# hellobertrand/zxc

Hardware: AMD Instinct MI355X
Metric: seekable decode GB/s (level 3, 64 KiB independent blocks, HBM-resident in/out) (higher is better)
Workload: dtype u8

## Files before the change

### zxc_amd/csrc/zxc_decode_kernel.hip

```cpp
#include "zxc_experiments.h"
#include <hip/hip_runtime.h>
#include <stdint.h>

#include "zxc_kernels.h"
#include "zxc_wave.h"

typedef unsigned __int128 u128;

#include "zxc_lds.h"

#define RING_BYTES 4096u
#define RING_MASK (RING_BYTES - 1u)
#define RING_WORDS (RING_BYTES / 4u)
#define REDIRECT_PASSES 2
#define SPARSE_MAX 8
#define TILE_MAX 3584u
#define LIT_MED 128u
#define MATCH_MED 128u
#define BYTEWISE_MAX 32u

#define E_DST_TOO_SMALL (-2)
#define E_SRC_TOO_SMALL (-3)
#define E_BAD_HEADER (-6)
#define E_BAD_CHECKSUM (-7)
// ... 1053 lines not shown
        return r;
    const uint64_t consumed = (uint64_t)lit_comp + tok_comp + (uint64_t)n_seq * (enc_off ? 1u : 2u);
    if (consumed > avail || avail - lit_comp < 32u) return r;
    if (enc_tok == 2u && (n_seq == 0u || n_seq > block_size / 5u + 16u || n_seq > PDIR_N_MAX || tok_comp < 128u || pdir_class(tok_comp - 128u) > 2u))
        return r;
    r.cls = ZXC_DEV_CLS_PRE;
    if (enc_lit == 2u) {
        r.lit16 = (16u + n_lit + 64u + 15u) >> 4;
        r.lit_cls = pdir_class(lit_comp - 128u);
        r.lit_at = 8u + 12u + desc;
        r.lit_psize = lit_comp;
        r.n_lit = n_lit;
    }
    if (enc_tok == 2u) {
        r.tok16 = (n_seq + 64u + 15u) >> 4;
        r.tok_cls = pdir_class(tok_comp - 128u);
        r.tok_at = 8u + 12u + desc + lit_comp;
        r.tok_psize = tok_comp;
        r.n_seq = n_seq;
    }
    return r;
}

template <bool PRE>
__device__ __forceinline__ void lean_one_block(const uint8_t* __restrict__ comp, const zxc_dev_job_t* __restrict__ jobs,
                                               uint8_t* __restrict__ out, int32_t* __restrict__ status, uint32_t block_size,
                                               uint32_t cap_override, uint32_t trailer_bytes, uint32_t b,
                                               const zxc_dev_pre_t* __restrict__ pre, const uint8_t* __restrict__ pscratch, LeanLds& L,
                                               int lane, const uint8_t* __restrict__ rle_slot, int rle_rc) {
    const uint32_t cap = cap_override ? cap_override : block_size + 2112u;
    const bool ck_here = !(trailer_bytes & ZXC_DEV_TRAILER_ELSEWHERE);
    trailer_bytes &= ~ZXC_DEV_TRAILER_ELSEWHERE;
#ifdef EXP_TIMES
    const uint64_t t_start = wall_clock64();
#endif
    const uint64_t comp_off = jobs[b].comp_off;
    const uint32_t src_sz = uni(jobs[b].comp_size);
    const uint32_t out_len = uni(jobs[b].out_len);
    const uint8_t* src = comp + comp_off;
    uint8_t* dst = out + jobs[b].out_off;
    int rc;
    if (src_sz < 8u) {
        rc = E_SRC_TOO_SMALL;
    } else {
        const uint32_t type = uni(ld8(src));
        const uint32_t comp_sz = uni(ld32(src + 3));
        if ((uint64_t)8u + comp_sz + trailer_bytes > src_sz) {
            rc = E_SRC_TOO_SMALL;
        } else if (trailer_bytes && ck_here && wave_checksum32(src + 8, comp_sz, lane) != uni(ld32(src + 8 + comp_sz))) {
            rc = E_BAD_CHECKSUM;
        } else if (PRE) {
            rc = type == 1u ? decode_lz_block_lean(src + 8, comp_sz, false, dst, out_len, cap, L, lane, pre + b, pscratch, false) : ZXC_DEV_E_INTERNAL;
        } else if (type == 1u || type == 2u) {
            rc = rle_slot ? rle_rc : 0;
            if (rc == 0) rc = decode_lz_block_lean(src + 8, comp_sz, type == 2u, dst, out_len, cap, L, lane, nullptr, pscratch, false,
                                                   rle_slot ? rle_slot + 16 : nullptr, rle_slot != nullptr);
        } else if (type == 0u) {
            if (comp_sz > cap) rc = E_DST_TOO_SMALL;
            else {
                const uint32_t n = comp_sz < out_len ? comp_sz : out_len;
                const uint8_t* s8 = src + 8;
                uint32_t i = 16u * lane;
                for (; i + 3072u + 16u <= n; i += 4096u) {
                    const v4u a0 = ld128(s8 + i), a1 = ld128(s8 + i + 1024u), a2 = ld128(s8 + i + 2048u),
                              a3 = ld128(s8 + i + 3072u);
                    *(v4u*)(dst + i) = a0;
                    *(v4u*)(dst + i + 1024u) = a1;
                    *(v4u*)(dst + i + 2048u) = a2;
                    *(v4u*)(dst + i + 3072u) = a3;
                }
                for (; i + 16u <= n; i += 1024u) *(v4u*)(dst + i) = ld128(s8 + i);
                const uint32_t tail = n & ~15u;
                if (tail + (uint32_t)lane < n) dst[tail + lane] = s8[tail + lane];
                rc = (int)comp_sz;
            }
        } else if (type == 255u) {
            rc = E_CORRUPT;
        } else {
            rc = E_BAD_BLOCK_TYPE;
        }
    }
#ifdef EXP_TIMES
    __builtin_amdgcn_s_waitcnt(0);
    {
        const uint64_t t_end = wall_clock64();
        rc = (int)((((uint32_t)(t_start >> 5) & 0xFFFFu) << 16) | (uint32_t)(((t_end - t_start) >> 5) & 0xFFFFu));
    }
#endif
    if (lane == 0) status[b] = rc == ZXC_DEV_DEFER ? ZXC_DEV_E_INTERNAL : rc;
}

extern "C" __global__ void __launch_bounds__(64, LEAN_WAVES_PER_SIMD)
zxc_decode_blocks_lean_kernel(const uint8_t* __restrict__ comp, const zxc_dev_job_t* __restrict__ jobs, uint32_t n_jobs,
                              uint8_t* __restrict__ out, int32_t* __restrict__ status, uint32_t block_size,
                              const uint32_t* __restrict__ order, uint32_t cap_override, uint32_t trailer_bytes,
                              const zxc_dev_pre_t* __restrict__ pre, const uint8_t* __restrict__ rscratch) {
    __shared__ LeanLds L;
    if (blockIdx.x >= n_jobs) return;
    const uint32_t b = order ? uni(order[blockIdx.x]) : blockIdx.x;
    const uint32_t cls = uni(pre[b].cls);
    if (cls != ZXC_DEV_CLS_LEAN && cls != ZXC_DEV_CLS_LEAN_RLE) return;
    const uint8_t* rle_slot = cls == ZXC_DEV_CLS_LEAN_RLE ? rscratch + 16ull * uni(pre[b].lit_off) : nullptr;
    const int rle_rc = cls == ZXC_DEV_CLS_LEAN_RLE ? (int)(int16_t)uni((uint32_t)(uint16_t)pre[b].rc_lit) : 0;
    lean_one_block<false>(comp, jobs, out, status, block_size, cap_override, trailer_bytes, b, nullptr, nullptr, L, threadIdx.x, rle_slot, rle_rc);
}

extern "C" __global__ void __launch_bounds__(64)
zxc_rle_expand_kernel(const uint8_t* __restrict__ comp, const zxc_dev_job_t* __restrict__ jobs, zxc_dev_pre_t* __restrict__ pre,
                      uint8_t* __restrict__ rscratch, const uint32_t* __restrict__ hdr, const uint32_t* __restrict__ entries_last) {
    const int lane = threadIdx.x;
    const uint32_t n = uni(hdr[0]);
    for (uint32_t i = blockIdx.x; i < n; i += gridDim.x) {
        const uint32_t b = uni(*(entries_last - i));
        const uint8_t* src = comp + jobs[b].comp_off;
        const uint32_t n_lit = uni(ld32(src + 12));
        int rc = 0;
        if (n_lit != 0u) rc = rle_expand(src + 8 + 16, uni(ld32(src + 20)), rscratch + 16ull * uni(pre[b].lit_off) + 16u, n_lit, lane);
        if (lane == 0) pre[b].rc_lit = (int16_t)rc;
    }
}

extern "C" __global__ void __launch_bounds__(64, LEAN_WAVES_PER_SIMD)
zxc_decode_blocks_lean_pre_kernel(const uint8_t* __restrict__ comp, const zxc_dev_job_t* __restrict__ jobs, uint8_t* __restrict__ out,
                                  int32_t* __restrict__ status, uint32_t block_size, uint32_t cap_override, uint32_t trailer_bytes,
                                  const zxc_dev_pre_t* __restrict__ pre, const uint8_t* __restrict__ pscratch,
                                  const uint32_t* __restrict__ hdr, const uint32_t* __restrict__ entries) {
    __shared__ LeanLds L;
    if (blockIdx.x >= uni(hdr[0])) return;
    lean_one_block<true>(comp, jobs, out, status, block_size, cap_override, trailer_bytes, uni(entries[blockIdx.x]), pre, pscratch, L, threadIdx.x, nullptr, 0);
}

extern "C" __global__ void __launch_bounds__(64)
zxc_block_checksum_kernel(const uint8_t* __restrict__ comp, const zxc_dev_job_t* __restrict__ jobs, uint32_t n_jobs,
                          const uint32_t* __restrict__ order, uint8_t* __restrict__ ck_bad) {
    const int lane = threadIdx.x;
    const uint32_t slot = blockIdx.x * 9u + (uint32_t)lane / 7u;
    const bool in = lane < 63 && slot < n_jobs;
    const uint32_t b = in ? (order ? order[slot] : slot) : 0u;
    const uint8_t* src = comp + jobs[b].comp_off;
    const uint32_t src_sz = in ? jobs[b].comp_size : 0u;
    uint32_t comp_sz = 0;
    bool on = false;
    if (src_sz >= 8u) {
        comp_sz = ld32(src + 3);
        on = (uint64_t)8u + comp_sz + 4u <= src_sz;
    }
    const uint32_t h = group_checksum32(src + 8, on ? comp_sz : 0u, lane, on);
    if (on && lane % 7 == 0) ck_bad[b] = h != ld32(src + 8 + comp_sz) ? 1u : 0u;
    else if (in && !on && lane % 7 == 0) ck_bad[b] = 0u;
}
extern "C" __global__ void __launch_bounds__(256)
zxc_checksum_merge_kernel(const uint8_t* __restrict__ ck_bad, int32_t* __restrict__ status, uint32_t n_jobs) {
    const uint32_t i = blockIdx.x * 256u + threadIdx.x;
    if (i < n_jobs && ck_bad[i]) status[i] = E_BAD_CHECKSUM;
}

__device__ __forceinline__ uint32_t order_bucket(const uint8_t* __restrict__ comp, const zxc_dev_job_t& j, uint32_t block_size) {
    uint32_t cost = 0;
    if (j.comp_size >= 8u + 12u) {
        const uint8_t* h = comp + j.comp_off;
        const uint32_t type = ld8(h);
        if (type == 1u || type == 2u) {
            const uint32_t n_seq = ld32(h + 8), n_lit = ld32(h + 12), enc_lit = ld8(h + 16), enc_tok = ld8(h + 17);
            cost = n_seq + (enc_tok == 2u ? n_seq : 0u) + (enc_lit == 1u ? n_lit >> 4 : 0u) + (enc_lit >= 2u ? n_lit >> 2 : 0u);
        }
    }
    const uint64_t q = (uint64_t)cost * 320u / block_size;
    return 63u - (q > 63u ? 63u : (uint32_t)q);
}

extern "C" __global__ void __launch_bounds__(256)
zxc_order_hist_kernel(const uint8_t* __restrict__ comp, const zxc_dev_job_t* __restrict__ jobs, uint32_t n_jobs,
                      uint32_t block_size, uint32_t* __restrict__ hist) {
    __shared__ uint32_t cnt[64];
    if (threadIdx.x < 64u) cnt[threadIdx.x] = 0;
    __syncthreads();
    const uint32_t i = blockIdx.x * 256u + threadIdx.x;
    if (i < n_jobs) atomicAdd(cnt + order_bucket(comp, jobs[i], block_size), 1u);
    __syncthreads();
    if (threadIdx.x < 64u && cnt[threadIdx.x]) atomicAdd(hist + threadIdx.x, cnt[threadIdx.x]);
}

extern "C" __global__ void __launch_bounds__(256)
zxc_order_scatter_kernel(const uint8_t* __restrict__ comp, const zxc_dev_job_t* __restrict__ jobs, uint32_t n_jobs,
                         uint32_t block_size, uint32_t* __restrict__ hist, uint32_t* __restrict__ order,
                         uint32_t* __restrict__ list, uint32_t trailer_bytes, zxc_dev_pre_t* __restrict__ pre,
                         uint32_t* __restrict__ ctl, uint32_t* __restrict__ pre_entries, zxc_dev_sec_t* __restrict__ secs,
                         uint32_t pscratch_cap16, uint32_t cap, uint32_t rscratch_cap16) {
    __shared__ uint32_t cnt[64], base[64];
    __shared__ uint32_t wg_cnt[8], wg_base[8];
    __shared__ uint32_t wg_fit, wg_rle_fit;
    if (threadIdx.x < 64u) cnt[threadIdx.x] = 0;
    if (threadIdx.x < 8u) wg_cnt[threadIdx.x] = 0;
    __syncthreads();
    const uint32_t i = blockIdx.x * 256u + threadIdx.x;
    uint32_t bk = 0, rank = 0;
    if (i < n_jobs) {
        bk = order_bucket(comp, jobs[i], block_size);
        rank = atomicAdd(cnt + bk, 1u);
    }
    __syncthreads();
    if (threadIdx.x < 64u) {
        uint32_t s = 0;
        for (uint32_t k = 0; k < threadIdx.x; k++) s += hist[k];
        base[threadIdx.x] = cnt[threadIdx.x] ? s + atomicAdd(hist + 64u + threadIdx.x, cnt[threadIdx.x]) : 0u;
    }
    __syncthreads();
    if (i < n_jobs) order[base[bk] + rank] = i;
    if (!list) return;
    BlockClass c = {ZXC_DEV_CLS_LEAN, 0, 0, 3, 3, 0, 0, 0, 0, 0, 0};
    uint32_t my_off = 0, my_pre = 0, my_full = 0, my_lit = 0, my_tok = 0;
    if (i < n_jobs) {
        c = classify_block(comp + jobs[i].comp_off, jobs[i].comp_size, trailer_bytes, block_size, cap);
        if (c.cls == ZXC_DEV_CLS_PRE) {
            my_off = atomicAdd(wg_cnt + 0, c.lit16 + c.tok16);
            my_pre = atomicAdd(wg_cnt + 1, 1u);
            if (c.lit_cls < 3u) my_lit = atomicAdd(wg_cnt + 3u + c.lit_cls, 1u);
            if (c.tok_cls < 3u) my_tok = atomicAdd(wg_cnt + 3u + c.tok_cls, 1u);
        } else if (c.cls == ZXC_DEV_CLS_FULL) {
            my_full = atomicAdd(wg_cnt + 2, 1u);
        } else if (c.cls == ZXC_DEV_CLS_LEAN_RLE) {
            my_off = atomicAdd(wg_cnt + 6, c.lit16);
            my_pre = atomicAdd(wg_cnt + 7, 1u);
        }
    }
    __syncthreads();
    if (threadIdx.x == 0) {
        bool rfit = rscratch_cap16 != 0u;
        wg_base[6] = 0;
        if (wg_cnt[7]) {
            atomicAdd(ctl + ZXC_DEV_CTL_RLE_WANTED, wg_cnt[6] + 1u);
            if (wg_cnt[6]) {
// ... 11 lines not shown
        }
        wg_rle_fit = rfit ? 1u : 0u;
        bool fit = true;
        wg_base[0] = 0;
        if (wg_cnt[0]) {
            uint32_t old = __hip_atomic_load(ctl + ZXC_DEV_CTL_CURSOR, __ATOMIC_RELAXED, __HIP_MEMORY_SCOPE_AGENT);
            for (;;) {
                if (old > pscratch_cap16) { fit = false; break; }
                const uint32_t seen = atomicCAS(ctl + ZXC_DEV_CTL_CURSOR, old, old + wg_cnt[0]);
                if (seen == old) { fit = (uint64_t)old + wg_cnt[0] <= pscratch_cap16; break; }
                old = seen;
            }
            wg_base[0] = old;
        }
        wg_fit = fit ? 1u : 0u;
        if (wg_cnt[1]) atomicAdd(ctl + ZXC_DEV_CTL_WANTED, wg_cnt[1]);
        if (fit) {
            wg_base[1] = wg_cnt[1] ? atomicAdd(ctl + ZXC_DEV_CTL_PRE, wg_cnt[1]) : 0u;
            wg_base[2] = wg_cnt[2] ? atomicAdd(list, wg_cnt[2]) : 0u;
            for (uint32_t k = 0; k < 3u; k++) wg_base[3u + k] = wg_cnt[3u + k] ? atomicAdd(ctl + ZXC_DEV_CTL_SEC + 2u * k, wg_cnt[3u + k]) : 0u;
        } else {
            wg_base[2] = atomicAdd(list, wg_cnt[2] + wg_cnt[1]);
        }
    }
    __syncthreads();
    if (i >= n_jobs) return;
    uint32_t cls = c.cls;
    if (cls == ZXC_DEV_CLS_PRE && !wg_fit) {
        cls = ZXC_DEV_CLS_FULL;
        my_full = wg_cnt[2] + my_pre;
    }
    if (cls == ZXC_DEV_CLS_LEAN_RLE) {
        if (wg_rle_fit) {
            pre_entries[n_jobs - 1u - (wg_base[7] + my_pre)] = i;
            pre[i].lit_off = wg_base[6] + my_off;
            pre[i].tok_off = 0;
            pre[i].rc_lit = 0;
            pre[i].rc_tok = 0;
            pre[i].cls = cls;
            return;
        }
        cls = ZXC_DEV_CLS_FULL;
        my_full = wg_cnt[2] - wg_cnt[7] + my_pre;
    }
    const uint32_t off = wg_base[0] + my_off;
    pre[i].lit_off = off;
    pre[i].tok_off = off + c.lit16;
    pre[i].rc_lit = 0;
    pre[i].rc_tok = 0;
    pre[i].cls = cls;
    if (cls == ZXC_DEV_CLS_FULL) {
        list[2u + wg_base[2] + my_full] = base[bk] + rank;
    } else if (cls == ZXC_DEV_CLS_PRE) {
        pre_entries[wg_base[1] + my_pre] = i;
        if (c.lit_cls < 3u) {
            zxc_dev_sec_t& s = secs[(size_t)c.lit_cls * 2u * n_jobs + wg_base[3u + c.lit_cls] + my_lit];
            s.src_off = jobs[i].comp_off + c.lit_at;
            s.psize = c.lit_psize;
            s.n = c.n_lit;
            s.out_off4 = 4u * off + 4u;
            s.rc_slot = 8u * i + 4u;
        }
        if (c.tok_cls < 3u) {
            zxc_dev_sec_t& s = secs[(size_t)c.tok_cls * 2u * n_jobs + wg_base[3u + c.tok_cls] + my_tok];
            s.src_off = jobs[i].comp_off + c.tok_at;
            s.psize = c.tok_psize;
            s.n = c.n_seq;
            s.out_off4 = 4u * (off + c.lit16);
            s.rc_slot = 8u * i + 5u;
        }
    }
}
```

### zxc_amd/csrc/zxc_dev.h

```cpp
#ifndef ZXC_DEV_H
#define ZXC_DEV_H
#include "../../include/zxc_mi355x.h"

#define ZXC_DEV_E_UNSUPPORTED (-101)
#define ZXC_DEV_DEFER (-103)
#define ZXC_DEV_E_INTERNAL (-102)

#define ZXC_DEV_CLS_LEAN 0u
#define ZXC_DEV_CLS_FULL 1u
#define ZXC_DEV_CLS_PRE 2u
#define ZXC_DEV_CLS_LEAN_RLE 3u
typedef struct {
    uint32_t lit_off;
    uint32_t tok_off;
    int16_t rc_lit, rc_tok;
    uint32_t cls;
} zxc_dev_pre_t;
typedef struct {
    uint64_t src_off;
    uint32_t psize, n;
    uint32_t out_off4;
    uint32_t rc_slot;
    uint32_t pad[2];
} zxc_dev_sec_t;
#define ZXC_DEV_TRAILER_ELSEWHERE 0x80000000u
#define ZXC_DEV_CTL_WORDS 32u
#define ZXC_DEV_CTL_PRE 0u
#define ZXC_DEV_CTL_CURSOR 2u
#define ZXC_DEV_CTL_WANTED 3u
#define ZXC_DEV_CTL_SEC 4u
#define ZXC_DEV_CTL_RLE_CURSOR 10u
#define ZXC_DEV_CTL_RLE_WANTED 11u
#define ZXC_DEV_CTL_RLE_LIST 12u

#define ZXC_DEV_SLOT_REGION(bs) ((bs) + 64u)
#define ZXC_DEV_SLOT_STRIDE(bs) ((2u * ZXC_DEV_SLOT_REGION(bs) + (bs) / 5u + 16u + 64u + 255u) & ~255u)

typedef struct { size_t list, order, ctl, pre_ent, secs, pre, ck_bad, words; } zxc_dev_ord_layout_t;
static inline zxc_dev_ord_layout_t zxc_dev_ord_layout(uint32_t n_jobs) {
    const size_t n = n_jobs, ctl = 130u + 2u * n, pre_ent = ctl + ZXC_DEV_CTL_WORDS, secs = (pre_ent + n + 7u) & ~(size_t)7u;
    const zxc_dev_ord_layout_t l = {128u, 130u + n, ctl, pre_ent, secs, secs + 48u * n, secs + 52u * n, secs + 52u * n + (n + 3u) / 4u};
    return l;
}

enum { ZXC_DEV_PLAN_FULL, ZXC_DEV_PLAN_DICT, ZXC_DEV_PLAN_TWO_PASS, ZXC_DEV_PLAN_TWO_PASS_PRE };
#define ZXC_DEV_DBG_NO_TWO_PASS 0x40000000u
#define ZXC_DEV_DBG_NO_ORDER 0x80000000u
typedef struct {
    uint32_t kind, ordered, ck_apart, trailer_bytes;
    uint64_t pscratch_bytes, rscratch_bytes;
} zxc_dev_plan_t;
typedef struct {
    uint32_t dict, cap_override, n_jobs, max_slots, debug, verify_trailer, block_size;
    uint32_t slot, helpers, hint, hint0, hint1;
    uint32_t ck_inline, no_rle_scratch, rle_lean_max_jobs, no_pre;
    uint32_t order_failed, pscratch_failed, rscratch_failed;
} zxc_dev_plan_in_t;

static inline zxc_dev_plan_t zxc_dev_plan_choose(const zxc_dev_plan_in_t* in) {
    const uint64_t gib = (uint64_t)1 << 30, n = in->n_jobs, bs = in->block_size;
    const int two_pass = !in->dict && !in->cap_override && !(in->debug & ZXC_DEV_DBG_NO_TWO_PASS);
    const int wants_order = two_pass || (in->n_jobs > in->max_slots && !(in->debug & ZXC_DEV_DBG_NO_ORDER));
    zxc_dev_plan_t p = {in->dict ? ZXC_DEV_PLAN_DICT : ZXC_DEV_PLAN_FULL, wants_order && in->slot && !in->order_failed, 0u,
                        in->verify_trailer ? 4u : 0u, 0u, 0u};
// ... 13 lines not shown
```

### zxc_amd/csrc/zxc_hip_shim.hip

```cpp
#include "zxc_experiments.h"
#include <hip/hip_runtime.h>
#include <pthread.h>
#include <stdint.h>
#include <stdlib.h>

#include "../../include/zxc_error.h"
#include "zxc_encode_levels.h"
#include "zxc_kernels.h"

#ifdef EXP_ENC_CLOCKS
extern "C" __attribute__((visibility("default"))) int zxc_mi355x_exp_enc_clocks(unsigned long long* out8) {
    unsigned long long* d = NULL;
    if (hipMalloc((void**)&d, 64) != hipSuccess) return -1;
    hipLaunchKernelGGL(zxc_enc_clk_read_kernel, dim3(1), dim3(64), 0, 0, d);
    const hipError_t e = hipMemcpy(out8, d, 64, hipMemcpyDeviceToHost);
    (void)hipFree(d);
    return e == hipSuccess ? 0 : -1;
}
#endif

#define ZXC_MAX_DEVICES 16
#define ZXC_RLE_LEAN_MAX_JOBS 16384u
#define ZXC_ORDER_STREAMS 16
#define ZXC_POOLS 10
struct Pool { uint8_t* scratch; uint32_t* busy; uint32_t n_slots; uint32_t stride; };
struct Ord {
    void* stream; int used; uint32_t* buf; size_t buf_cap; hipStream_t aux, aux2; hipEvent_t fork, join, join2, small_done;
    uint32_t* hint; uint8_t* pscratch; size_t pscratch_cap; uint8_t* rscratch; size_t rscratch_cap;
};
static struct {
    Pool pool[ZXC_POOLS];
    int cus, wg_per_cu;
    Ord ord[ZXC_ORDER_STREAMS];
} g_dev[ZXC_MAX_DEVICES];
static pthread_mutex_t g_lock = PTHREAD_MUTEX_INITIALIZER;

#ifdef ZXC_EXPERIMENT
static uint32_t g_debug_flags = 0;
#else
#define g_debug_flags 0u
#endif

static int current_device(void) {
    int d = -1;
    if (hipGetDevice(&d) != hipSuccess || d < 0 || d >= ZXC_MAX_DEVICES) return -1;
    return d;
}

extern "C" {

#ifdef ZXC_EXPERIMENT
// ... 138 lines not shown
static Ord* claim_slot(int dev, void* stream) {
    Ord* ord = g_dev[dev].ord;
    for (int i = 0; i < ZXC_ORDER_STREAMS; i++)
        if (ord[i].used && ord[i].stream == stream) return &ord[i];
    for (int i = 0; i < ZXC_ORDER_STREAMS; i++)
        if (!ord[i].used) {
            ord[i].used = 1, ord[i].stream = stream;
            if (ord[i].hint) { ord[i].hint[0] = 0xFFFFFFFFu; ord[i].hint[1] = 0u; }
            return &ord[i];
        }
    return NULL;
}

static void make_helpers(Ord& o) {
    if (o.aux) return;
    if (hipStreamCreateWithFlags(&o.aux, hipStreamNonBlocking) != hipSuccess) { o.aux = NULL; return; }
    const unsigned f = hipEventDisableTiming;
    if (hipStreamCreateWithFlags(&o.aux2, hipStreamNonBlocking) != hipSuccess) { (void)hipStreamDestroy(o.aux); o.aux = NULL; return; }
    if (hipEventCreateWithFlags(&o.fork, f) != hipSuccess || hipEventCreateWithFlags(&o.join, f) != hipSuccess ||
        hipEventCreateWithFlags(&o.join2, f) != hipSuccess || hipEventCreateWithFlags(&o.small_done, f) != hipSuccess) {
        (void)hipStreamDestroy(o.aux), (void)hipStreamDestroy(o.aux2);
        o.aux = NULL;
    } else if (!o.hint) {
        if (hipHostMalloc((void**)&o.hint, 64, hipHostMallocDefault) == hipSuccess) { o.hint[0] = 0xFFFFFFFFu; o.hint[1] = 0u; }
        else o.hint = NULL;
    }
}

static bool grow(void** p, size_t* cap, size_t bytes) {
    if (*cap >= bytes) return true;
    if (*p) (void)hipFree(*p);
    *cap = 0;
    if (hipMalloc(p, bytes) != hipSuccess) { *p = NULL; return false; }
    *cap = bytes;
    return true;
}

struct Launch {
    const uint8_t* comp; const zxc_dev_job_t* jobs; uint32_t n; uint8_t* out; int32_t* status; uint32_t bs, cap_override;
    zxc_dev_plan_t plan; hipStream_t s0; const Pool* pool; uint32_t max_slots, cus; Ord* o;
    uint32_t *order, *list, *ctl, *pre_entries; zxc_dev_sec_t* secs; zxc_dev_pre_t* pre;
    uint8_t *ck_bad, *pscratch, *rscratch; uint32_t pscratch_cap16, rscratch_cap16;
};

static void order_pass(const Launch& L) {
    const uint32_t g = (L.n + 255u) / 256u;
    hipLaunchKernelGGL(zxc_order_hist_kernel, dim3(g), dim3(256), 0, L.s0, L.comp, L.jobs, L.n, L.bs, L.o->buf);
    hipLaunchKernelGGL(zxc_order_scatter_kernel, dim3(g), dim3(256), 0, L.s0, L.comp, L.jobs, L.n, L.bs, L.o->buf, L.order, L.list,
                       L.plan.trailer_bytes & ~ZXC_DEV_TRAILER_ELSEWHERE, L.pre, L.ctl, L.pre_entries, L.secs, L.pscratch_cap16,
                       L.cap_override ? L.cap_override : L.bs + 2112u, L.rscratch_cap16);
    if (L.ctl && L.o->hint) {
        (void)hipMemcpyAsync(L.o->hint, L.ctl + ZXC_DEV_CTL_WANTED, 4, hipMemcpyDeviceToHost, L.s0);
        (void)hipMemcpyAsync(L.o->hint + 1, L.ctl + ZXC_DEV_CTL_RLE_WANTED, 4, hipMemcpyDeviceToHost, L.s0);
    }
}

static void launch_full(const Launch& L, hipStream_t st, uint32_t grid) {
    hipLaunchKernelGGL(zxc_decode_blocks_kernel, dim3(grid), dim3(64), 0, st, L.comp, L.jobs, L.n, L.out, L.status, L.bs, L.plan.trailer_bytes,
                       L.pool->scratch, L.pool->stride, g_debug_flags, L.pool->busy, L.pool->n_slots, L.order, L.cap_override, L.list);
}

static void launch_rle(const Launch& L, hipStream_t st) {
    if (!L.rscratch_cap16) return;
    hipLaunchKernelGGL(zxc_rle_expand_kernel, dim3(L.n < 8u * L.cus ? L.n : 8u * L.cus), dim3(64), 0, st, L.comp, L.jobs, L.pre,
                       L.rscratch, L.ctl + ZXC_DEV_CTL_RLE_LIST, L.pre_entries + L.n - 1u);
}

static bool fork_to(Ord& o, hipStream_t h) { return hipStreamWaitEvent(h, o.fork, 0) == hipSuccess; }
static int fail(Ord& o) { (void)hipStreamSynchronize(o.aux), (void)hipStreamSynchronize(o.aux2); return ZXC_ERROR_GPU_UNAVAILABLE; }
static int join(Ord& o, hipStream_t s0, bool aux, bool aux2) {
    if ((aux && (hipEventRecord(o.join, o.aux) != hipSuccess || hipStreamWaitEvent(s0, o.join, 0) != hipSuccess)) ||
        (aux2 && (hipEventRecord(o.join2, o.aux2) != hipSuccess || hipStreamWaitEvent(s0, o.join2, 0) != hipSuccess)))
        return fail(o);
    return ZXC_OK;
}

static int enqueue_two_pass(const Launch& L) {
// ... 38 lines not shown
    if (n_jobs == 0) return ZXC_OK;
    if (!d_comp || !d_jobs || !d_out || !d_status) return ZXC_ERROR_NULL_INPUT;
    if (block_size < (1u << 12) || block_size > (1u << 21) || (block_size & (block_size - 1u))) return ZXC_ERROR_BAD_BLOCK_SIZE;
    const int dev = current_device();
    if (dev < 0) return ZXC_ERROR_GPU_UNAVAILABLE;
    zxc_dev_plan_in_t in = {(uint32_t)(d_dict || d_dict_huf), cap_override, n_jobs, 0u, g_debug_flags, (uint32_t)(verify_trailer != 0), block_size};
    in.rle_lean_max_jobs = ZXC_RLE_LEAN_MAX_JOBS;
    in.ck_inline = getenv("ZXC_MI355X_CK_INLINE") != NULL, in.no_rle_scratch = getenv("ZXC_MI355X_NO_RLE_SCRATCH") != NULL;
#ifdef EXP_NO_PRE
    in.no_pre = 1;
#endif
    struct Unlock { ~Unlock() { pthread_mutex_unlock(&g_lock); } } unlock_on_return;
    pthread_mutex_lock(&g_lock);
    Pool* pool;
    if (const int rc = setup_pool(dev, block_size, &pool, &in.max_slots)) return rc;
    in.slot = in.helpers = 1;
    const zxc_dev_plan_t could = zxc_dev_plan_choose(&in);
    Ord* o = could.ordered ? claim_slot(dev, stream) : NULL;
    if (o && could.kind >= ZXC_DEV_PLAN_TWO_PASS) make_helpers(*o);
    in.slot = o != NULL; in.helpers = o && o->aux; in.hint = o && o->hint;
    if (in.hint) { in.hint0 = *(volatile uint32_t*)o->hint; in.hint1 = *(volatile uint32_t*)(o->hint + 1); }
    zxc_dev_plan_t plan = zxc_dev_plan_choose(&in);
    const hipStream_t s0 = (hipStream_t)stream; const zxc_dev_ord_layout_t at = zxc_dev_ord_layout(n_jobs);
    if (plan.ordered) in.order_failed = !grow((void**)&o->buf, &o->buf_cap, at.words * 4u);
    if (plan.pscratch_bytes) in.pscratch_failed = !grow((void**)&o->pscratch, &o->pscratch_cap, plan.pscratch_bytes);
    if (plan.rscratch_bytes) in.rscratch_failed = !grow((void**)&o->rscratch, &o->rscratch_cap, plan.rscratch_bytes);
    if (plan.ordered && !in.order_failed)
        in.order_failed = hipMemsetAsync(o->buf, 0, 130u * 4u, s0) != hipSuccess ||
                          hipMemsetAsync(o->buf + at.ctl, 0, ZXC_DEV_CTL_WORDS * 4u, s0) != hipSuccess;
    plan = zxc_dev_plan_choose(&in);
    Launch L = {(const uint8_t*)d_comp, d_jobs, n_jobs, (uint8_t*)d_out, d_status, block_size, cap_override, plan, s0, pool,
                in.max_slots, (uint32_t)g_dev[dev].cus, o};
    if (plan.ordered) L.order = o->buf + at.order;
    if (plan.kind >= ZXC_DEV_PLAN_TWO_PASS) {
        L.list = o->buf + at.list; L.ctl = o->buf + at.ctl; L.pre_entries = o->buf + at.pre_ent;
        L.secs = (zxc_dev_sec_t*)(o->buf + at.secs); L.pre = (zxc_dev_pre_t*)(o->buf + at.pre); L.ck_bad = (uint8_t*)(o->buf + at.ck_bad);
        if (plan.pscratch_bytes) { L.pscratch = o->pscratch; L.pscratch_cap16 = (uint32_t)(o->pscratch_cap >> 4); }
        if (plan.rscratch_bytes) { L.rscratch = o->rscratch; L.rscratch_cap16 = (uint32_t)(o->rscratch_cap >> 4); }
    }
    if (plan.ordered) order_pass(L);
    if (plan.kind == ZXC_DEV_PLAN_TWO_PASS || plan.kind == ZXC_DEV_PLAN_TWO_PASS_PRE) {
        if (const int rc = plan.kind == ZXC_DEV_PLAN_TWO_PASS ? enqueue_two_pass(L) : enqueue_two_pass_pre(L)) return rc;
    } else if (plan.kind == ZXC_DEV_PLAN_DICT)
        hipLaunchKernelGGL(zxc_decode_blocks_dict_kernel, dim3(n_jobs), dim3(64), 0, s0, L.comp, d_jobs, n_jobs, L.out, d_status, block_size,
                           plan.trailer_bytes, pool->scratch, pool->stride, g_debug_flags, pool->busy, pool->n_slots, L.order, cap_override,
                           (const uint8_t*)d_dict, dict_size, (const uint8_t*)d_dict_huf);
    else
        launch_full(L, s0, n_jobs);
    return hipGetLastError() == hipSuccess ? ZXC_OK : ZXC_ERROR_GPU_UNAVAILABLE;
}

int zxc_mi355x_decode_blocks_device(const void* d_comp, const zxc_dev_job_t* d_jobs, uint32_t n_jobs, void* d_out,
// ... 91 lines not shown
```

### zxc_amd/csrc/zxc_kernels.h

```cpp
#ifndef ZXC_KERNELS_H
#define ZXC_KERNELS_H
#include <hip/hip_runtime.h>
#include <stdint.h>

#include "zxc_dev.h"

#define PDIR_SMALL_THREADS 128
#define PDIR_MEDIUM_THREADS 256
#define PDIR_LARGE_THREADS 512

extern "C" __global__ void zxc_decode_blocks_kernel(const uint8_t* comp, const zxc_dev_job_t* jobs, uint32_t n_jobs,
                                                    uint8_t* out, int32_t* status, uint32_t block_size,
                                                    uint32_t trailer_bytes, uint8_t* scratch, uint32_t scratch_stride, uint32_t dbg,
                                                    uint32_t* slot_busy, uint32_t n_slots, const uint32_t* order,
                                                    uint32_t cap_override, uint32_t* list);
extern "C" __global__ void zxc_decode_blocks_dict_kernel(const uint8_t* comp, const zxc_dev_job_t* jobs, uint32_t n_jobs,
                                                         uint8_t* out, int32_t* status, uint32_t block_size,
                                                         uint32_t trailer_bytes, uint8_t* scratch, uint32_t scratch_stride,
                                                         uint32_t dbg, uint32_t* slot_busy, uint32_t n_slots,
                                                         const uint32_t* order, uint32_t cap_override, const uint8_t* dict,
                                                         uint32_t dict_size, const uint8_t* dict_huf);
extern "C" __global__ void zxc_decode_blocks_lean_kernel(const uint8_t* comp, const zxc_dev_job_t* jobs, uint32_t n_jobs,
                                                         uint8_t* out, int32_t* status, uint32_t block_size,
                                                         const uint32_t* order, uint32_t cap_override, uint32_t trailer_bytes,
                                                         const zxc_dev_pre_t* pre, const uint8_t* rscratch);
extern "C" __global__ void zxc_decode_blocks_lean_pre_kernel(const uint8_t* comp, const zxc_dev_job_t* jobs, uint8_t* out, int32_t* status,
                                                             uint32_t block_size, uint32_t cap_override, uint32_t trailer_bytes,
                                                             const zxc_dev_pre_t* pre, const uint8_t* pscratch, const uint32_t* hdr,
                                                             const uint32_t* entries);
extern "C" __global__ void zxc_rle_expand_kernel(const uint8_t* comp, const zxc_dev_job_t* jobs, zxc_dev_pre_t* pre, uint8_t* rscratch,
                                                 const uint32_t* hdr, const uint32_t* entries_last);
extern "C" __global__ void zxc_order_hist_kernel(const uint8_t* comp, const zxc_dev_job_t* jobs, uint32_t n_jobs,
                                                 uint32_t block_size, uint32_t* hist);
extern "C" __global__ void zxc_order_scatter_kernel(const uint8_t* comp, const zxc_dev_job_t* jobs, uint32_t n_jobs,
                                                    uint32_t block_size, uint32_t* hist, uint32_t* order, uint32_t* list, uint32_t trailer_bytes,
                                                    zxc_dev_pre_t* pre, uint32_t* ctl, uint32_t* pre_entries, zxc_dev_sec_t* secs,
                                                    uint32_t pscratch_cap16, uint32_t cap, uint32_t rscratch_cap16);
#define ZXC_SECTIONS_KERNEL(name)                                                                                              \
    extern "C" __global__ void name(const uint8_t* comp, const zxc_dev_sec_t* secs, uint32_t* hdr, zxc_dev_pre_t* pre, uint8_t* pscratch)
ZXC_SECTIONS_KERNEL(zxc_pivco_sections_small_kernel);
ZXC_SECTIONS_KERNEL(zxc_pivco_sections_medium_kernel);
ZXC_SECTIONS_KERNEL(zxc_pivco_sections_large_kernel);
#undef ZXC_SECTIONS_KERNEL
extern "C" __global__ void zxc_block_checksum_kernel(const uint8_t* comp, const zxc_dev_job_t* jobs, uint32_t n_jobs, const uint32_t* order, uint8_t* ck_bad);
extern "C" __global__ void zxc_checksum_merge_kernel(const uint8_t* ck_bad, int32_t* status, uint32_t n_jobs);

#define ZXC_ENCODE_DECL(name)                                                                                          \
    extern "C" __global__ void name(const uint8_t* src, uint64_t src_size, uint32_t block_size, uint8_t* slots,        \
                                    uint32_t slot_stride, uint32_t* sizes, uint32_t n_blocks, uint32_t with_checksum,  \
                                    uint32_t depth, uint32_t sufficient, uint32_t lazy, uint32_t dict_size,        \
                                    uint8_t* huf_scratch, uint32_t huf)
ZXC_ENCODE_DECL(zxc_encode_blocks_kernel_l1);
ZXC_ENCODE_DECL(zxc_encode_blocks_kernel_l2);
ZXC_ENCODE_DECL(zxc_encode_blocks_kernel_l3);
ZXC_ENCODE_DECL(zxc_encode_blocks_kernel_l4);
ZXC_ENCODE_DECL(zxc_encode_blocks_kernel_l57);
ZXC_ENCODE_DECL(zxc_encode_blocks_kernel_l67);
#undef ZXC_ENCODE_DECL
extern "C" __global__ void zxc_prepend_dict_kernel(const uint8_t* src, uint64_t src_size, uint32_t block_size, const uint8_t* dict,
                                                   uint32_t dict_size, uint8_t* work, uint32_t n_blocks);
// ... 8 lines not shown
```

### zxc_amd/csrc/zxc_seq_lean.inc

```
struct __attribute__((aligned(16))) LeanLds : RingLds {
    uint32_t vval[64];
    uint32_t vpos[66];
};
#define LEAN_VARINTS 62u
#define LEAN_TILE_MAX (RING_BYTES - 1056u)

#ifdef ASM_MARKERS
#define PHM(i) asm volatile("; PHMARK " #i)
#else
#define PHM(i) do { } while (0)
#endif

__device__ __forceinline__ uint32_t mbcnt64(uint64_t m) {
    return __builtin_amdgcn_mbcnt_hi((uint32_t)(m >> 32), __builtin_amdgcn_mbcnt_lo((uint32_t)m, 0u));
}

template <bool GHI>
__device__ __forceinline__ int run_sequences_lean(const LzStreams& S, uint8_t* __restrict__ dst, uint32_t out_len, uint32_t cap,
                                                  LeanLds& L, int lane, const bool strict) {
    const uint32_t n_total = S.n_seq + 1u;
    const uint32_t n_lit = S.n_lit;
    const uint32_t RW = GHI ? 513u : 33u, RD = GHI ? 2112u : 168u, RLM = GHI ? 1016u : 56u;
    const uint32_t trig_d = strict ? 0u : 3u * RW + 32u, trig_l = strict ? 0u : 3u * (GHI ? 255u : 15u);
    bool carry4x = true;
// ... 416 lines not shown
        PHM(14);
        if (!strict && ((seq_base + k) & 3u) != 0u) {
            const uint32_t g = (seq_base + k) & ~3u;
            if (g >= seq_base) {
                const uint32_t ge = (uint32_t)__builtin_amdgcn_readlane((int)est, (int)(g - seq_base)),
                               gl = (uint32_t)__builtin_amdgcn_readlane((int)lst, (int)(g - seq_base));
                carry4x = ge + RD < cap && n_lit > RLM && gl < n_lit - RLM;
            }
        }
        seq_base += k;
        raw_t = nraw_t;
        raw_o = nraw_o;
        xw = nxw;
        wave_lds_fence();
    }
    flush_to(L, O, p, lane);
    if ((p & 15u) != 0u && lane == 0) {
        const uint32_t cs = p & ~15u;
        for (uint32_t kk = 0; cs + kk < p && cs + kk < out_len; kk++) dst[cs + kk] = (uint8_t)ring_rd8(L, cs + kk);
    }
    return (int)p;
}

__device__ __forceinline__ int decode_lz_block_lean(const uint8_t* data, uint32_t comp_sz, bool ghi, uint8_t* dst, uint32_t out_len,
                                                    uint32_t cap, LeanLds& L, int lane, const zxc_dev_pre_t* pd,
                                                    const uint8_t* pscratch, const bool strict, const uint8_t* rle_lit = nullptr,
                                                    const bool rle_ok = false) {
    if (comp_sz < 12u) return E_BAD_HEADER;
    LzStreams S;
    S.dict = nullptr;
    S.dict_size = 0;
    S.n_seq = uni(ld32(data));
    S.n_lit = uni(ld32(data + 4));
    const uint32_t enc_lit = uni(ld8(data + 8)), enc_tok = uni(ld8(data + 9)), enc_off = uni(ld8(data + 11));
    const uint32_t avail = comp_sz - 12u;
    if (ghi) {
        if (enc_lit != 0u || enc_tok != 0u) return E_CORRUPT;
        const uint64_t consumed = (uint64_t)S.n_lit + 4ull * S.n_seq;
        if (consumed > avail || avail - S.n_lit < 32u) return E_CORRUPT;
        S.lit = data + 12;
        S.tok = S.lit + S.n_lit;
        S.offs = nullptr;
        S.off8 = 0;
        S.ext = S.tok + 4ull * S.n_seq;
        S.ext_size = avail - (uint32_t)consumed;
        return run_sequences_lean<true>(S, dst, out_len, cap, L, lane, strict);
    }
    if (!pd && rle_ok) {
        const uint32_t lit_comp = uni(ld32(data + 12));
        const uint8_t* d = data + 16;
        const uint32_t sz_off = S.n_seq * (enc_off ? 1u : 2u);
        S.lit = S.n_lit ? rle_lit : d;
        S.tok = d + lit_comp;
        S.offs = S.tok + S.n_seq;
        S.off8 = enc_off;
        S.ext = S.offs + sz_off;
        S.ext_size = comp_sz - 16u - (lit_comp + S.n_seq + sz_off);
// ... 32 lines not shown
```

Before: 1011.

## Precompute per-block header records in order pass and write hint from device

The order-scatter kernel now gathers each block's job fields and LZ header (sizes, sequence/literal counts, encodings) into a packed record stored in sorted order. The lean decode kernel reads that one record instead of chasing order, then jobs, then the compressed header, which shortens its serial dependent-load chain at kernel start. The scatter kernel also uses a last-block ticket to reset the histogram and write the host hint straight into mapped coherent host memory, replacing two D2H memcpys and per-call memsets. This adds record writes to the scatter pass, makes the lean kernel require an order buffer, and moves buffer clearing into the kernels.

```diff
diff --git a/zxc_amd/csrc/zxc_decode_kernel.hip b/zxc_amd/csrc/zxc_decode_kernel.hip
--- a/zxc_amd/csrc/zxc_decode_kernel.hip
+++ b/zxc_amd/csrc/zxc_decode_kernel.hip
@@ -1099,10 +1099,34 @@
     return r;
 }
 
+struct LeanHdr {
+    uint32_t b, encs, src_sz, comp_sz, out_len, n_seq, n_lit;
+    uint64_t comp_off, out_off;
+};
+__device__ __forceinline__ LeanHdr lean_hdr_load(const uint8_t* __restrict__ comp, const zxc_dev_job_t* __restrict__ jobs, uint32_t b,
+                                                 uint32_t trailer_bytes) {
+    LeanHdr h = {b, 0u, jobs[b].comp_size, 0u, jobs[b].out_len, 0u, 0u, jobs[b].comp_off, jobs[b].out_off};
+    const uint8_t* src = comp + h.comp_off;
+    if (h.src_sz >= 8u) {
+        h.encs = ld8(src);
+        h.comp_sz = ld32(src + 3);
+        if (h.comp_sz >= 12u && (uint64_t)8u + h.comp_sz + trailer_bytes <= h.src_sz) {
+            h.n_seq = ld32(src + 8);
+            h.n_lit = ld32(src + 12);
+            h.encs |= ld8(src + 16) << 8 | ld8(src + 17) << 16 | ld8(src + 19) << 24;
+        }
+    }
+    return h;
+}
+__device__ __forceinline__ uint64_t uni64(uint64_t v) { return (uint64_t)uni((uint32_t)(v >> 32)) << 32 | uni((uint32_t)v); }
+__device__ __forceinline__ LeanHdr lean_hdr_uniform(const LeanHdr& v) {
+    const LeanHdr h = {uni(v.b), uni(v.encs), uni(v.src_sz), uni(v.comp_sz), uni(v.out_len), uni(v.n_seq), uni(v.n_lit), uni64(v.comp_off), uni64(v.out_off)};
+    return h;
+}
+
 template <bool PRE>
-__device__ __forceinline__ void lean_one_block(const uint8_t* __restrict__ comp, const zxc_dev_job_t* __restrict__ jobs,
-                                               uint8_t* __restrict__ out, int32_t* __restrict__ status, uint32_t block_size,
-                                               uint32_t cap_override, uint32_t trailer_bytes, uint32_t b,
+__device__ __forceinline__ void lean_one_block(const uint8_t* __restrict__ comp, uint8_t* __restrict__ out, int32_t* __restrict__ status,
+                                               uint32_t block_size, uint32_t cap_override, uint32_t trailer_bytes, const LeanHdr& h,
                                                const zxc_dev_pre_t* __restrict__ pre, const uint8_t* __restrict__ pscratch, LeanLds& L,
                                                int lane, const uint8_t* __restrict__ rle_slot, int rle_rc) {
     const uint32_t cap = cap_override ? cap_override : block_size + 2112u;
@@ -1111,27 +1135,25 @@
 #ifdef EXP_TIMES
     const uint64_t t_start = wall_clock64();
 #endif
-    const uint64_t comp_off = jobs[b].comp_off;
-    const uint32_t src_sz = uni(jobs[b].comp_size);
-    const uint32_t out_len = uni(jobs[b].out_len);
-    const uint8_t* src = comp + comp_off;
-    uint8_t* dst = out + jobs[b].out_off;
+    const uint32_t b = h.b, src_sz = h.src_sz, out_len = h.out_len;
+    const uint8_t* src = comp + h.comp_off;
+    uint8_t* dst = out + h.out_off;
     int rc;
     if (src_sz < 8u) {
         rc = E_SRC_TOO_SMALL;
     } else {
-        const uint32_t type = uni(ld8(src));
-        const uint32_t comp_sz = uni(ld32(src + 3));
+        const uint32_t type = h.encs & 255u;
+        const uint32_t comp_sz = h.comp_sz;
         if ((uint64_t)8u + comp_sz + trailer_bytes > src_sz) {
             rc = E_SRC_TOO_SMALL;
         } else if (trailer_bytes && ck_here && wave_checksum32(src + 8, comp_sz, lane) != uni(ld32(src + 8 + comp_sz))) {
             rc = E_BAD_CHECKSUM;
         } else if (PRE) {
-            rc = type == 1u ? decode_lz_block_lean(src + 8, comp_sz, false, dst, out_len, cap, L, lane, pre + b, pscratch, false) : ZXC_DEV_E_INTERNAL;
+            rc = type == 1u ? decode_lz_block_lean(src + 8, comp_sz, h.n_seq, h.n_lit, h.encs, false, dst, out_len, cap, L, lane, pre + b, pscratch, false) : ZXC_DEV_E_INTERNAL;
         } else if (type == 1u || type == 2u) {
             rc = rle_slot ? rle_rc : 0;
-            if (rc == 0) rc = decode_lz_block_lean(src + 8, comp_sz, type == 2u, dst, out_len, cap, L, lane, nullptr, pscratch, false,
-                                                   rle_slot ? rle_slot + 16 : nullptr, rle_slot != nullptr);
+            if (rc == 0) rc = decode_lz_block_lean(src + 8, comp_sz, h.n_seq, h.n_lit, h.encs, type == 2u, dst, out_len, cap, L, lane, nullptr, pscratch,
+                                                   false, rle_slot ? rle_slot + 16 : nullptr, rle_slot != nullptr);
         } else if (type == 0u) {
             if (comp_sz > cap) rc = E_DST_TOO_SMALL;
             else {
@@ -1174,12 +1196,20 @@
                               const zxc_dev_pre_t* __restrict__ pre, const uint8_t* __restrict__ rscratch) {
     __shared__ LeanLds L;
     if (blockIdx.x >= n_jobs) return;
-    const uint32_t b = order ? uni(order[blockIdx.x]) : blockIdx.x;
-    const uint32_t cls = uni(pre[b].cls);
+    if (!order) {
+        if (threadIdx.x == 0) status[blockIdx.x] = ZXC_DEV_E_INTERNAL;
+        return;
+    }
+    const zxc_dev_rec_t* __restrict__ r =
+        reinterpret_cast<const zxc_dev_rec_t*>(order - zxc_dev_ord_layout(n_jobs).order + zxc_dev_ord_rec(n_jobs)) + blockIdx.x;
+    const LeanHdr h = {uni(r->job), uni(r->hdr), uni(r->comp_size), uni(r->comp_sz), uni(r->out_len), uni(r->n_seq), uni(r->n_lit),
+                       uni64(r->comp_off), uni64(r->out_off)};
+    const uint32_t co = uni(r->cls_off);
+    const uint32_t cls = co >> 30, lit_off = co & 0x3FFFFFFFu;
     if (cls != ZXC_DEV_CLS_LEAN && cls != ZXC_DEV_CLS_LEAN_RLE) return;
-    const uint8_t* rle_slot = cls == ZXC_DEV_CLS_LEAN_RLE ? rscratch + 16ull * uni(pre[b].lit_off) : nullptr;
-    const int rle_rc = cls == ZXC_DEV_CLS_LEAN_RLE ? (int)(int16_t)uni((uint32_t)(uint16_t)pre[b].rc_lit) : 0;
-    lean_one_block<false>(comp, jobs, out, status, block_size, cap_override, trailer_bytes, b, nullptr, nullptr, L, threadIdx.x, rle_slot, rle_rc);
+    const uint8_t* rle_slot = cls == ZXC_DEV_CLS_LEAN_RLE ? rscratch + 16ull * lit_off : nullptr;
+    const int rle_rc = cls == ZXC_DEV_CLS_LEAN_RLE ? (int)(int16_t)uni((uint32_t)(uint16_t)pre[h.b].rc_lit) : 0;
+    lean_one_block<false>(comp, out, status, block_size, cap_override, trailer_bytes, h, nullptr, nullptr, L, threadIdx.x, rle_slot, rle_rc);
 }
 
 extern "C" __global__ void __launch_bounds__(64)
@@ -1204,7 +1234,8 @@
                                   const uint32_t* __restrict__ hdr, const uint32_t* __restrict__ entries) {
     __shared__ LeanLds L;
     if (blockIdx.x >= uni(hdr[0])) return;
-    lean_one_block<true>(comp, jobs, out, status, block_size, cap_override, trailer_bytes, uni(entries[blockIdx.x]), pre, pscratch, L, threadIdx.x, nullptr, 0);
+    const LeanHdr h = lean_hdr_uniform(lean_hdr_load(comp, jobs, uni(entries[blockIdx.x]), trailer_bytes & ~ZXC_DEV_TRAILER_ELSEWHERE));
+    lean_one_block<true>(comp, out, status, block_size, cap_override, trailer_bytes, h, pre, pscratch, L, threadIdx.x, nullptr, 0);
 }
 
 extern "C" __global__ void __launch_bounds__(64)
@@ -1251,6 +1282,10 @@
                       uint32_t block_size, uint32_t* __restrict__ hist) {
     __shared__ uint32_t cnt[64];
     if (threadIdx.x < 64u) cnt[threadIdx.x] = 0;
+    if (blockIdx.x == 0) {
+        if (threadIdx.x < 66u) hist[64u + threadIdx.x] = 0;
+        else if (threadIdx.x < 66u + ZXC_DEV_CTL_WORDS) hist[zxc_dev_ord_layout(n_jobs).ctl + threadIdx.x - 66u] = 0;
+    }
     __syncthreads();
     const uint32_t i = blockIdx.x * 256u + threadIdx.x;
     if (i < n_jobs) atomicAdd(cnt + order_bucket(comp, jobs[i], block_size), 1u);
@@ -1258,12 +1293,29 @@
     if (threadIdx.x < 64u && cnt[threadIdx.x]) atomicAdd(hist + threadIdx.x, cnt[threadIdx.x]);
 }
 
-extern "C" __global__ void __launch_bounds__(256)
-zxc_order_scatter_kernel(const uint8_t* __restrict__ comp, const zxc_dev_job_t* __restrict__ jobs, uint32_t n_jobs,
+#ifdef __HIP__
+#define ORDER_THREADFENCE() __threadfence()
+#define ORDER_SCOPE_SYSTEM __HIP_MEMORY_SCOPE_SYSTEM
+#else
+#define ORDER_THREADFENCE() do { } while (0)
+#define ORDER_SCOPE_SYSTEM 0
+#endif
+__device__ __forceinline__ void order_pass_done(uint32_t* __restrict__ hist, uint32_t* __restrict__ ctl, bool two_pass, uint32_t* __restrict__ hint) {
+    ORDER_THREADFENCE();
+    if (atomicAdd(ctl + ZXC_DEV_CTL_TICKET, 1u) != gridDim.x - 1u) return;
+    ORDER_THREADFENCE();
+    if (two_pass && hint) {
+        __hip_atomic_store(hint, __hip_atomic_load(ctl + ZXC_DEV_CTL_WANTED, __ATOMIC_RELAXED, __HIP_MEMORY_SCOPE_AGENT), __ATOMIC_RELAXED, ORDER_SCOPE_SYSTEM);
+        __hip_atomic_store(hint + 1, __hip_atomic_load(ctl + ZXC_DEV_CTL_RLE_WANTED, __ATOMIC_RELAXED, __HIP_MEMORY_SCOPE_AGENT), __ATOMIC_RELAXED, ORDER_SCOPE_SYSTEM);
+    }
+    for (uint32_t k = 0; k < 64u; k++) hist[k] = 0;
+}
+
+__device__ __forceinline__ void order_scatter(const uint8_t* __restrict__ comp, const zxc_dev_job_t* __restrict__ jobs, uint32_t n_jobs,
                          uint32_t block_size, uint32_t* __restrict__ hist, uint32_t* __restrict__ order,
                          uint32_t* __restrict__ list, uint32_t trailer_bytes, zxc_dev_pre_t* __restrict__ pre,
                          uint32_t* __restrict__ ctl, uint32_t* __restrict__ pre_entries, zxc_dev_sec_t* __restrict__ secs,
-                         uint32_t pscratch_cap16, uint32_t cap, uint32_t rscratch_cap16) {
+                         uint32_t pscratch_cap16, uint32_t cap, uint32_t rscratch_cap16, uint32_t* __restrict__ hint) {
     __shared__ uint32_t cnt[64], base[64];
     __shared__ uint32_t wg_cnt[8], wg_base[8];
     __shared__ uint32_t wg_fit, wg_rle_fit;
@@ -1284,7 +1336,10 @@
     }
     __syncthreads();
     if (i < n_jobs) order[base[bk] + rank] = i;
-    if (!list) return;
+    if (!list) {
+        if (threadIdx.x == 0) order_pass_done(hist, hist + zxc_dev_ord_layout(n_jobs).ctl, false, nullptr);
+        return;
+    }
     BlockClass c = {ZXC_DEV_CLS_LEAN, 0, 0, 3, 3, 0, 0, 0, 0, 0, 0};
     uint32_t my_off = 0, my_pre = 0, my_full = 0, my_lit = 0, my_tok = 0;
     if (i < n_jobs) {
@@ -1342,9 +1397,14 @@
         } else {
             wg_base[2] = atomicAdd(list, wg_cnt[2] + wg_cnt[1]);
         }
+        order_pass_done(hist, ctl, true, hint);
     }
     __syncthreads();
     if (i >= n_jobs) return;
+    const LeanHdr h = lean_hdr_load(comp, jobs, i, trailer_bytes);
+    zxc_dev_rec_t* __restrict__ rec = reinterpret_cast<zxc_dev_rec_t*>(hist + zxc_dev_ord_rec(n_jobs)) + (base[bk] + rank);
+    rec->job = i, rec->hdr = h.encs, rec->comp_off = h.comp_off, rec->comp_size = h.src_sz, rec->comp_sz = h.comp_sz;
+    rec->out_off = h.out_off, rec->out_len = h.out_len, rec->n_seq = h.n_seq, rec->n_lit = h.n_lit;
     uint32_t cls = c.cls;
     if (cls == ZXC_DEV_CLS_PRE && !wg_fit) {
         cls = ZXC_DEV_CLS_FULL;
@@ -1358,6 +1418,7 @@
             pre[i].rc_lit = 0;
             pre[i].rc_tok = 0;
             pre[i].cls = cls;
+            rec->cls_off = cls << 30 | (wg_base[6] + my_off);
             return;
         }
         cls = ZXC_DEV_CLS_FULL;
@@ -1369,6 +1430,7 @@
     pre[i].rc_lit = 0;
     pre[i].rc_tok = 0;
     pre[i].cls = cls;
+    rec->cls_off = cls << 30;
     if (cls == ZXC_DEV_CLS_FULL) {
         list[2u + wg_base[2] + my_full] = base[bk] + rank;
     } else if (cls == ZXC_DEV_CLS_PRE) {
@@ -1391,3 +1453,22 @@
         }
     }
 }
+
+extern "C" __global__ void __launch_bounds__(256)
+zxc_order_scatter_kernel(const uint8_t* __restrict__ comp, const zxc_dev_job_t* __restrict__ jobs, uint32_t n_jobs,
+                         uint32_t block_size, uint32_t* __restrict__ hist, uint32_t* __restrict__ order,
+                         uint32_t* __restrict__ list, uint32_t trailer_bytes, zxc_dev_pre_t* __restrict__ pre,
+                         uint32_t* __restrict__ ctl, uint32_t* __restrict__ pre_entries, zxc_dev_sec_t* __restrict__ secs,
+                         uint32_t pscratch_cap16, uint32_t cap, uint32_t rscratch_cap16) {
+    order_scatter(comp, jobs, n_jobs, block_size, hist, order, list, trailer_bytes, pre, ctl, pre_entries, secs, pscratch_cap16, cap,
+                  rscratch_cap16, nullptr);
+}
+extern "C" __global__ void __launch_bounds__(256)
+zxc_order_scatter_hint_kernel(const uint8_t* __restrict__ comp, const zxc_dev_job_t* __restrict__ jobs, uint32_t n_jobs,
+                              uint32_t block_size, uint32_t* __restrict__ hist, uint32_t* __restrict__ order,
+                              uint32_t* __restrict__ list, uint32_t trailer_bytes, zxc_dev_pre_t* __restrict__ pre,
+                              uint32_t* __restrict__ ctl, uint32_t* __restrict__ pre_entries, zxc_dev_sec_t* __restrict__ secs,
+                              uint32_t pscratch_cap16, uint32_t cap, uint32_t rscratch_cap16, uint32_t* __restrict__ hint) {
+    order_scatter(comp, jobs, n_jobs, block_size, hist, order, list, trailer_bytes, pre, ctl, pre_entries, secs, pscratch_cap16, cap,
+                  rscratch_cap16, hint);
+}
diff --git a/zxc_amd/csrc/zxc_dev.h b/zxc_amd/csrc/zxc_dev.h
--- a/zxc_amd/csrc/zxc_dev.h
+++ b/zxc_amd/csrc/zxc_dev.h
@@ -32,14 +32,37 @@
 #define ZXC_DEV_CTL_RLE_CURSOR 10u
 #define ZXC_DEV_CTL_RLE_WANTED 11u
 #define ZXC_DEV_CTL_RLE_LIST 12u
+#define ZXC_DEV_CTL_TICKET 14u
+
+typedef struct {
+    uint32_t job;
+    uint32_t hdr;
+    uint64_t comp_off;
+    uint32_t comp_size;
+    uint32_t comp_sz;
+    uint64_t out_off;
+    uint32_t out_len, n_seq, n_lit;
+    uint32_t cls_off;
+} zxc_dev_rec_t;
+#define ZXC_DEV_REC_WORDS 12u
 
 #define ZXC_DEV_SLOT_REGION(bs) ((bs) + 64u)
 #define ZXC_DEV_SLOT_STRIDE(bs) ((2u * ZXC_DEV_SLOT_REGION(bs) + (bs) / 5u + 16u + 64u + 255u) & ~255u)
 
+#ifdef __HIP__
+#define ZXC_DEV_HD __host__ __device__
+#else
+#define ZXC_DEV_HD
+#endif
 typedef struct { size_t list, order, ctl, pre_ent, secs, pre, ck_bad, words; } zxc_dev_ord_layout_t;
-static inline zxc_dev_ord_layout_t zxc_dev_ord_layout(uint32_t n_jobs) {
+ZXC_DEV_HD static inline size_t zxc_dev_ord_rec(uint32_t n_jobs) {
+    const size_t n = n_jobs, secs = (130u + 2u * n + ZXC_DEV_CTL_WORDS + n + 7u) & ~(size_t)7u;
+    return (secs + 52u * n + (n + 3u) / 4u + 7u) & ~(size_t)7u;
+}
+ZXC_DEV_HD static inline zxc_dev_ord_layout_t zxc_dev_ord_layout(uint32_t n_jobs) {
     const size_t n = n_jobs, ctl = 130u + 2u * n, pre_ent = ctl + ZXC_DEV_CTL_WORDS, secs = (pre_ent + n + 7u) & ~(size_t)7u;
-    const zxc_dev_ord_layout_t l = {128u, 130u + n, ctl, pre_ent, secs, secs + 48u * n, secs + 52u * n, secs + 52u * n + (n + 3u) / 4u};
+    const zxc_dev_ord_layout_t l = {128u, 130u + n, ctl, pre_ent, secs, secs + 48u * n, secs + 52u * n,
+                                    zxc_dev_ord_rec(n_jobs) + ZXC_DEV_REC_WORDS * n};
     return l;
 }
 
diff --git a/zxc_amd/csrc/zxc_hip_shim.hip b/zxc_amd/csrc/zxc_hip_shim.hip
--- a/zxc_amd/csrc/zxc_hip_shim.hip
+++ b/zxc_amd/csrc/zxc_hip_shim.hip
@@ -26,7 +26,7 @@
 struct Pool { uint8_t* scratch; uint32_t* busy; uint32_t n_slots; uint32_t stride; };
 struct Ord {
     void* stream; int used; uint32_t* buf; size_t buf_cap; hipStream_t aux, aux2; hipEvent_t fork, join, join2, small_done;
-    uint32_t* hint; uint8_t* pscratch; size_t pscratch_cap; uint8_t* rscratch; size_t rscratch_cap;
+    uint32_t *hint, *hint_dev; uint8_t* pscratch; size_t pscratch_cap; uint8_t* rscratch; size_t rscratch_cap;
 };
 static struct {
     Pool pool[ZXC_POOLS];
@@ -211,8 +211,9 @@
         (void)hipStreamDestroy(o.aux), (void)hipStreamDestroy(o.aux2);
         o.aux = NULL;
     } else if (!o.hint) {
-        if (hipHostMalloc((void**)&o.hint, 64, hipHostMallocDefault) == hipSuccess) { o.hint[0] = 0xFFFFFFFFu; o.hint[1] = 0u; }
-        else o.hint = NULL;
+        if (hipHostMalloc((void**)&o.hint, 64, hipHostMallocMapped | hipHostMallocCoherent) != hipSuccess) o.hint = NULL;
+        else if (hipHostGetDevicePointer((void**)&o.hint_dev, o.hint, 0) != hipSuccess) { (void)hipHostFree(o.hint); o.hint = o.hint_dev = NULL; }
+        else { o.hint[0] = 0xFFFFFFFFu; o.hint[1] = 0u; }
     }
 }
 
@@ -235,13 +236,9 @@
 static void order_pass(const Launch& L) {
     const uint32_t g = (L.n + 255u) / 256u;
     hipLaunchKernelGGL(zxc_order_hist_kernel, dim3(g), dim3(256), 0, L.s0, L.comp, L.jobs, L.n, L.bs, L.o->buf);
-    hipLaunchKernelGGL(zxc_order_scatter_kernel, dim3(g), dim3(256), 0, L.s0, L.comp, L.jobs, L.n, L.bs, L.o->buf, L.order, L.list,
+    hipLaunchKernelGGL(zxc_order_scatter_hint_kernel, dim3(g), dim3(256), 0, L.s0, L.comp, L.jobs, L.n, L.bs, L.o->buf, L.order, L.list,
                        L.plan.trailer_bytes & ~ZXC_DEV_TRAILER_ELSEWHERE, L.pre, L.ctl, L.pre_entries, L.secs, L.pscratch_cap16,
-                       L.cap_override ? L.cap_override : L.bs + 2112u, L.rscratch_cap16);
-    if (L.ctl && L.o->hint) {
-        (void)hipMemcpyAsync(L.o->hint, L.ctl + ZXC_DEV_CTL_WANTED, 4, hipMemcpyDeviceToHost, L.s0);
-        (void)hipMemcpyAsync(L.o->hint + 1, L.ctl + ZXC_DEV_CTL_RLE_WANTED, 4, hipMemcpyDeviceToHost, L.s0);
-    }
+                       L.cap_override ? L.cap_override : L.bs + 2112u, L.rscratch_cap16, L.ctl ? L.o->hint_dev : (uint32_t*)NULL);
 }
 
 static void launch_full(const Launch& L, hipStream_t st, uint32_t grid) {
@@ -326,12 +323,11 @@
     if (in.hint) { in.hint0 = *(volatile uint32_t*)o->hint; in.hint1 = *(volatile uint32_t*)(o->hint + 1); }
     zxc_dev_plan_t plan = zxc_dev_plan_choose(&in);
     const hipStream_t s0 = (hipStream_t)stream; const zxc_dev_ord_layout_t at = zxc_dev_ord_layout(n_jobs);
-    if (plan.ordered) in.order_failed = !grow((void**)&o->buf, &o->buf_cap, at.words * 4u);
+    if (plan.ordered && o->buf_cap < at.words * 4u)
+        if ((in.order_failed = !grow((void**)&o->buf, &o->buf_cap, at.words * 4u) || hipMemsetAsync(o->buf, 0, 64u * 4u, s0) != hipSuccess))
+            o->buf_cap = 0;
     if (plan.pscratch_bytes) in.pscratch_failed = !grow((void**)&o->pscratch, &o->pscratch_cap, plan.pscratch_bytes);
     if (plan.rscratch_bytes) in.rscratch_failed = !grow((void**)&o->rscratch, &o->rscratch_cap, plan.rscratch_bytes);
-    if (plan.ordered && !in.order_failed)
-        in.order_failed = hipMemsetAsync(o->buf, 0, 130u * 4u, s0) != hipSuccess ||
-                          hipMemsetAsync(o->buf + at.ctl, 0, ZXC_DEV_CTL_WORDS * 4u, s0) != hipSuccess;
     plan = zxc_dev_plan_choose(&in);
     Launch L = {(const uint8_t*)d_comp, d_jobs, n_jobs, (uint8_t*)d_out, d_status, block_size, cap_override, plan, s0, pool,
                 in.max_slots, (uint32_t)g_dev[dev].cus, o};
diff --git a/zxc_amd/csrc/zxc_kernels.h b/zxc_amd/csrc/zxc_kernels.h
--- a/zxc_amd/csrc/zxc_kernels.h
+++ b/zxc_amd/csrc/zxc_kernels.h
@@ -36,6 +36,10 @@
                                                     uint32_t block_size, uint32_t* hist, uint32_t* order, uint32_t* list, uint32_t trailer_bytes,
                                                     zxc_dev_pre_t* pre, uint32_t* ctl, uint32_t* pre_entries, zxc_dev_sec_t* secs,
                                                     uint32_t pscratch_cap16, uint32_t cap, uint32_t rscratch_cap16);
+extern "C" __global__ void zxc_order_scatter_hint_kernel(const uint8_t* comp, const zxc_dev_job_t* jobs, uint32_t n_jobs,
+                                                         uint32_t block_size, uint32_t* hist, uint32_t* order, uint32_t* list, uint32_t trailer_bytes,
+                                                         zxc_dev_pre_t* pre, uint32_t* ctl, uint32_t* pre_entries, zxc_dev_sec_t* secs,
+                                                         uint32_t pscratch_cap16, uint32_t cap, uint32_t rscratch_cap16, uint32_t* hint);
 #define ZXC_SECTIONS_KERNEL(name)                                                                                              \
     extern "C" __global__ void name(const uint8_t* comp, const zxc_dev_sec_t* secs, uint32_t* hdr, zxc_dev_pre_t* pre, uint8_t* pscratch)
 ZXC_SECTIONS_KERNEL(zxc_pivco_sections_small_kernel);
diff --git a/zxc_amd/csrc/zxc_seq_lean.inc b/zxc_amd/csrc/zxc_seq_lean.inc
--- a/zxc_amd/csrc/zxc_seq_lean.inc
+++ b/zxc_amd/csrc/zxc_seq_lean.inc
@@ -462,7 +462,8 @@
     return (int)p;
 }
 
-__device__ __forceinline__ int decode_lz_block_lean(const uint8_t* data, uint32_t comp_sz, bool ghi, uint8_t* dst, uint32_t out_len,
+__device__ __forceinline__ int decode_lz_block_lean(const uint8_t* data, uint32_t comp_sz, uint32_t n_seq, uint32_t n_lit, uint32_t encs,
+                                                    bool ghi, uint8_t* dst, uint32_t out_len,
                                                     uint32_t cap, LeanLds& L, int lane, const zxc_dev_pre_t* pd,
                                                     const uint8_t* pscratch, const bool strict, const uint8_t* rle_lit = nullptr,
                                                     const bool rle_ok = false) {
@@ -470,9 +471,9 @@
     LzStreams S;
     S.dict = nullptr;
     S.dict_size = 0;
-    S.n_seq = uni(ld32(data));
-    S.n_lit = uni(ld32(data + 4));
-    const uint32_t enc_lit = uni(ld8(data + 8)), enc_tok = uni(ld8(data + 9)), enc_off = uni(ld8(data + 11));
+    S.n_seq = n_seq;
+    S.n_lit = n_lit;
+    const uint32_t enc_lit = (encs >> 8) & 255u, enc_tok = (encs >> 16) & 255u, enc_off = encs >> 24;
     const uint32_t avail = comp_sz - 12u;
     if (ghi) {
         if (enc_lit != 0u || enc_tok != 0u) return E_CORRUPT;
```

After: 1008. About the same (-0.2%).
